# xiuqhou/Salience-DETR

Measured on AMD Instinct MI355X. Metric: images/s (whole node) + ms/encoder-layer, ResNet50 800x1333, higher is better.
Workload: dtype bf16; 1 GPU; salience_detr_resnet50_800_1333 bf16 inference, batch=2 per MI355X: pyramid flatten + hierarchical salience filtering + 6-layer salience encoder (MSDA); batch_per_gpu=2, global_batch=2, parallelism=replicas, images sharded across GPUs, no data-path collective, hipgraph=True, hipgraph_nodes=45, hipgraph_memset_nodes=0, world_size=1, backend=none (single process)

## Files before the change

include/salience_hip.h:

```cpp
#ifndef SALIENCE_HIP_H_
#define SALIENCE_HIP_H_

#include <stddef.h>
#include <stdint.h>

#ifdef __cplusplus
extern "C" {
#endif

typedef struct ihipStream_t *sdetr_stream_t;

#define SDETR_ABI_VERSION 1
#define SDETR_EINVAL (-1)

#define SDETR_F32 0
#define SDETR_BF16 1
#define SDETR_F16 2
#define SDETR_I64 3


int sdetr_abi_version(void);
const char *sdetr_last_error(void);

int sdetr_msda_im2col_f32(sdetr_stream_t stream, const float *data_value,
// ... 240 lines not shown
                                           int64_t mask_row_stride, const float *fill_value, int batch_size, int n, int k,
                                           int slices, int64_t index_offset, float *out_score, int64_t *out_index,
                                           int64_t out_row_stride, void *workspace, size_t workspace_bytes,
                                           const sdetr_rank_job *rank, const sdetr_finalize_job *finalize,
                                           int *jobs_carried);
int sdetr_stage1_x3_with_jobs(
    sdetr_stream_t stream, const float *x, int64_t x_batch_stride, int64_t x_row_stride, int batch_size, int tokens,
    int channels, const void *enc_weight_x3, const float *enc_bias, const float *enc_norm_weight,
    const float *enc_norm_bias, float enc_norm_eps, const float *row_scale, const float *coarse_score, int coarse_h,
    int coarse_w, int level_h, int level_w, const float *alpha, const float *norm_weight, const float *norm_bias,
    float norm_eps, const void *weight_x3, const float *bias, float *memory_out, int64_t memory_batch_stride,
    float *z_local, float *partial_sums, const void *vp_x, const void *vp_packed_weight, const float *vp_bias_padded,
    const uint8_t *vp_pad_mask, int vp_batch_size, int vp_spatial_size, int vp_num_heads, int vp_num_groups,
    void *vp_dst, int vp_dst_dtype, const sdetr_bordered_layout *vp_bordered, const sdetr_rank_job *rank,
    const sdetr_finalize_job *finalize);
int sdetr_salience_head_hoist_x3(
    sdetr_stream_t stream, const float *x, int64_t x_batch_stride, int64_t x_row_stride, int batch_size, int tokens,
    int channels, const void *enc_weight_x3, const float *enc_bias, const float *enc_norm_weight,
    const float *enc_norm_bias, float enc_norm_eps, const float *norm_weight, const void *weight_x3, float *memory_out,
    int64_t memory_batch_stride, float *g_out, int64_t g_batch_stride, float *sigma_out, int64_t sigma_batch_stride,
    const void *vp_x, const void *vp_packed_weight, const float *vp_bias_padded, const uint8_t *vp_pad_mask,
    int vp_batch_size, int vp_spatial_size, int vp_num_heads, int vp_num_groups, void *vp_dst, int vp_dst_dtype,
    const sdetr_bordered_layout *vp_bordered, const sdetr_finalize_job *finalize);
int sdetr_salience_head_modulate(sdetr_stream_t stream, const float *g, int64_t g_batch_stride, const float *sigma,
                                 int64_t sigma_batch_stride, int batch_size, int tokens, const float *row_scale,
                                 const float *coarse_score, int coarse_h, int coarse_w, int level_h, int level_w,
                                 const float *alpha, float norm_eps, const float *c0, float *z_local, float *partial_sums,
                                 const sdetr_rank_job *rank, const sdetr_finalize_job *finalize, float *score_min_init);
int sdetr_stage1_x3_with_value_proj(
    sdetr_stream_t stream, const float *x, int64_t x_batch_stride, int64_t x_row_stride, int batch_size, int tokens,
    int channels, const void *enc_weight_x3, const float *enc_bias, const float *enc_norm_weight,
    const float *enc_norm_bias, float enc_norm_eps, const float *row_scale, const float *coarse_score, int coarse_h,
    int coarse_w, int level_h, int level_w, const float *alpha, const float *norm_weight, const float *norm_bias,
    float norm_eps, const void *weight_x3, const float *bias, float *memory_out, int64_t memory_batch_stride,
    float *z_local, float *partial_sums, const void *vp_x, const void *vp_packed_weight, const float *vp_bias_padded,
    const uint8_t *vp_pad_mask, int vp_batch_size, int vp_spatial_size, int vp_num_heads, int vp_num_groups,
    void *vp_dst, int vp_dst_dtype, const sdetr_bordered_layout *vp_bordered);
int sdetr_salience_head_const(sdetr_stream_t stream, const float *partial_sums, int batch_size, int tokens,
                              const float *weight2, const float *bias2, float *const_workspace, float *score_min);
int sdetr_stage2_with_value_proj(sdetr_stream_t stream, const float *z_local, int batch_size, int tokens,
                                 const float *weight2_local_packed, const float *weight3_packed, const float *bias3,
                                 const float *weight4, const float *bias4, const float *const_workspace, float *score,
                                 float *score_flat, int64_t score_flat_stride, float *score_min, const void *vp_x,
                                 const void *vp_packed_weight, const float *vp_bias_padded, const uint8_t *vp_pad_mask,
                                 int vp_batch_size, int vp_spatial_size, int vp_num_heads, int vp_num_groups,
                                 void *vp_dst, int vp_dst_dtype, const sdetr_bordered_layout *vp_bordered,
// ... 340 lines not shown
```

salience_detr_amd/_hip.py:

```python
import ctypes
import os
import threading
from typing import Optional

import torch

_HERE = os.path.dirname(os.path.abspath(__file__))
LIB_PATH = os.path.join(_HERE, "libsalience_hip.so")
F16_LIB_PATH = os.path.join(_HERE, "libsalience_hip_f16.so")

F32, BF16, F16, I64 = 0, 1, 2, 3
EINVAL = -1
ACT16 = (torch.bfloat16, torch.float16)

_lib = None
_lib_f16 = None
_tls = threading.local()


def is_act16(dt) -> bool:
    return dt in ACT16

_i = ctypes.c_int

# ... 114 lines not shown
    "sdetr_pyramid_flatten": (_i, [_p, _i, _p, _p, _p, _p, _p, _p, _i, _i, _i, _p, _p, _p, _p, _p, _p, _p]),
    "sdetr_class_max_times": (_i, [_p, _p, _i, _p, _i64, _i, _i, _i, _p]),
    "sdetr_layernorm": (_i, [_p, _p, _p, _i, _i64, _i64, _i64, _i64, _p, _p, _p, _p, _i, ctypes.c_float, _i, _i, _i, _p, _i,
                             _p, _i64, _i]),
    "sdetr_advance_rows": (_i, [_p, _p, _p, _p, _p, _p, _i64, _p, _i, _i, _i, _i, _i, _i]),
    "sdetr_select_stack": (_i, [_p, _p, _i64, _p, _i64, _p, _i, _i, _i, _i, _p]),
    "sdetr_encoder_finalize_sorted": (_i, [_p, _p, _p, _p, _p, _p, _p, _i, _i, _i, _i, _i, _i, _p]),
    "sdetr_encoder_finalize": (_i, [_p, _p, _p, _p, _p, _p, _p, _i, _i, _i, _i, _i, _i, _p]),
    "sdetr_column_mean_f32": (_i, [_p, _p, _i64, _i64, _i, _i, _i, _p]),
    "sdetr_pack_linear_f32": (_i, [_p, _p, _i64, _i, _i, _p]),
    "sdetr_salience_head_blocks": (_i, [_i, _i]),
    "sdetr_salience_head_stage1": (_i, [_p, _p, _i64, _i64, _i, _i, _i, _p, _p, _p, _p, ctypes.c_float, _p, _p, _i, _i,
                                        _i, _i, _p, _p, _p, ctypes.c_float, _p, _p, _p, _i64, _p, _p]),
    "sdetr_salience_head_stage1_x3": (_i, [_p, _p, _i64, _i64, _i, _i, _i, _p, _p, _p, _p, ctypes.c_float, _p, _p, _i, _i,
                                        _i, _i, _p, _p, _p, ctypes.c_float, _p, _p, _p, _i64, _p, _p]),
    "sdetr_salience_head_const": (_i, [_p, _p, _i, _i, _p, _p, _p, _p]),
    "sdetr_stage2_with_value_proj": (_i, [_p, _p, _i, _i, _p, _p, _p, _p, _p, _p, _p, _p, _i64, _p,
                                          _p, _p, _p, _p, _i, _i, _i, _i, _p, _i, _p, _p, _p, _p, _p]),
    "sdetr_stage1_x3_with_value_proj": (_i, [_p, _p, _i64, _i64, _i, _i, _i, _p, _p, _p, _p, ctypes.c_float, _p, _p, _i, _i,
                                        _i, _i, _p, _p, _p, ctypes.c_float, _p, _p, _p, _i64, _p, _p,
                                             _p, _p, _p, _p, _i, _i, _i, _i, _p, _i, _p]),
    "sdetr_salience_head_hoist_x3": (_i, [_p, _p, _i64, _i64, _i, _i, _i, _p, _p, _p, _p, ctypes.c_float, _p, _p, _p, _i64, _p,
                                          _i64, _p, _i64, _p, _p, _p, _p, _i, _i, _i, _i, _p, _i, _p, _p]),
    "sdetr_salience_head_modulate": (_i, [_p, _p, _i64, _p, _i64, _i, _i, _p, _p, _i, _i, _i, _i, _p, ctypes.c_float, _p, _p, _p,
                                          _p, _p, _p]),
    "sdetr_stage1_x3_with_jobs": (_i, [_p, _p, _i64, _i64, _i, _i, _i, _p, _p, _p, _p, ctypes.c_float, _p, _p, _i, _i,
                                        _i, _i, _p, _p, _p, ctypes.c_float, _p, _p, _p, _i64, _p, _p,
                                             _p, _p, _p, _p, _i, _i, _i, _i, _p, _i, _p, _p, _p]),
    "sdetr_pack_linear_bf16x3": (_i, [_p, _p, _i64, _i, _i, _p]),
    "sdetr_salience_head_stage2": (_i, [_p, _p, _p, _i, _i, _p, _p, _p, _p, _p, _p, _p, _p, _p, _p, _i64, _p, _p, _i]),
    "sdetr_ffn_packed_bytes": (_i64, [_i]),
    "sdetr_ffn_pack_bf16": (_i, [_p, _p, _p, _i, _i, _p]),
    "sdetr_ffn_auto_splits": (_i, [_i, _i]),
    "sdetr_ffn_workspace_bytes": (_i64, [_i, _i]),
    "sdetr_ffn_fused_advance_bf16": (_i, [_p, _p, _p, _p, _p, _p, _p, ctypes.c_float, _i, _i, _i, _i, _i, _p, _i64, _p, _p, _p, _p,
                                          _i64, _p, _i, _i, _i]),
    "sdetr_attn_tail_packed_bytes": (_i64, []),
    "sdetr_attn_tail_pack_bf16": (_i, [_p, _p, _i, _p]),
    "sdetr_attn_tail_ffn_advance_bf16": (_i, [_p, _p, _p, _p, _p, _p, _p, ctypes.c_float, _p, _p, _p, _p, ctypes.c_float, _i, _i,
                                              _i, _i, _i, _p, _i64, _p, _p, _p, _p, _i64, _p, _i, _i, _i, _p, _p, _i64, _p]),
    "sdetr_class_head_packed_bytes": (_i64, []),
    "sdetr_class_head_pack_bf16": (_i, [_p, _p, _i, _i, _p]),
    "sdetr_gemm_x3_presplit": (_i, [_p, _p, _i64, _i, _i, _i, _p]),
    "sdetr_gemm_x3_f32": (_i, [_p, _p, _i64, _i, _p, _i64, _i, _p, _i64, _i, _i, _i, _p, _i, _p]),
    "sdetr_gemm_x3_epilogue_f32": (_i, [_p, _p, _i64, _i, _p, _i64, _i, _p, _i64, _i, _i, _i, _p, _i, _p, _i, _p, _i64]),
    "sdetr_topk_attention_with_projection_bf16": (_i, [_p, _p, _i64, _p, _i64, _p, _i, _i, _i, _p, _p, _p, _p, _p, _p,
# ... 125 lines not shown
```

salience_detr_amd/csrc/salience_head.hip:

```cpp
#include <cstdlib>

#include "common.h"

#include "salience_head_core.h"

namespace sdetr {

__global__ void __launch_bounds__(512, 2) salience_head_stage1_x3_kernel(Stage1Args p)
{
    stage1_x3_body(p, (int)blockIdx.x, (int)blockIdx.y);
}


template <int RT, int WAVES = 4>
__global__ void __launch_bounds__(64 * WAVES, WAVES == 8 ? 2 : (RT == 2 ? 2 : 4)) salience_head_stage1_kernel(Stage1Args p)
{
    constexpr int TM = 32 * RT, THREADS = 64 * WAVES, CT = 8 / WAVES;
    static_assert(TM * 64 % THREADS == 0 && THREADS % TM == 0, "tile / block shape");
    extern __shared__ __attribute__((aligned(16))) float smem[];
    float *tile = smem;
    float *par = smem + TM * kXS;
    float *srow = par + kParRows * kC;
    const int tid = threadIdx.x, lane = tid & 63, wave = tid >> 6;
    const int b = blockIdx.y, blk = blockIdx.x;
    const int t0 = blk * TM;
    const int nvalid = min(TM, p.n - t0);
    const int n0 = wave * (32 * CT);
    const bool with_enc = p.w_enc != nullptr;

    WeightStream<CT, 4> ws;
    ws.start(with_enc ? p.w_enc : p.w1, kC, kC / 8, n0, lane);

    {
        const float *xb = p.x + (int64_t)b * p.x_batch_stride + (int64_t)t0 * p.x_row_stride;
        constexpr int NL = TM * 64 / THREADS;
// ... 331 lines not shown
        return fail("salience_head_stage1_x3: NULL pointer");
    if (enc_weight_x3 && (!enc_bias || !enc_norm_weight || !enc_norm_bias))
        return fail("salience_head_stage1_x3: enc_output parameters incomplete");
    if (row_scale && coarse_score) return fail("salience_head_stage1_x3: give row_scale OR coarse_score");
    if (coarse_score && ((int64_t)level_h * level_w != tokens || coarse_h <= 0 || coarse_w <= 0))
        return fail("salience_head_stage1_x3: level %dx%d does not cover %d tokens", level_h, level_w, tokens);
    if ((x_row_stride % 4) || (x_batch_stride % 4)) return fail("salience_head_stage1_x3: rows must be 16-byte aligned");
    if (stage1_block_tokens(batch_size, tokens) != 32)
        return fail("salience_head_stage1_x3: 32-token blocks only (unset SDETR_HEAD_ROWTILES)");
    Stage1Args a;
    a.x = x; a.x_batch_stride = x_batch_stride; a.x_row_stride = x_row_stride;
    a.w_enc = reinterpret_cast<const float4 *>(enc_weight_x3);
    a.b_enc = enc_bias; a.g_enc = enc_norm_weight; a.beta_enc = enc_norm_bias; a.eps_enc = enc_norm_eps;
    a.row_scale = row_scale; a.coarse = coarse_score; a.ch = coarse_h; a.cw = coarse_w; a.h = level_h; a.w = level_w;
    a.alpha = alpha; a.g1 = norm_weight; a.beta1 = norm_bias; a.eps1 = norm_eps;
    a.w1 = reinterpret_cast<const float4 *>(weight_x3); a.b1 = bias;
    a.memory_out = enc_weight_x3 ? memory_out : nullptr; a.mem_batch_stride = memory_batch_stride;
    a.z_local = z_local; a.partial = partial_sums; a.n = tokens; a.nblk = (tokens + 31) / 32;
    hipLaunchKernelGGL(salience_head_stage1_x3_kernel, dim3((unsigned)a.nblk, (unsigned)batch_size), dim3(512),
                       (size_t)stage1_x3_lds_bytes(), static_cast<hipStream_t>(stream), a);
    return check_launch("salience_head_stage1_x3");
}

extern "C" int sdetr_salience_head_const(sdetr_stream_t stream, const float *partial_sums, int batch_size, int tokens,
                                         const float *weight2, const float *bias2, float *const_workspace,
                                         float *score_min)
{
    if (batch_size < 0 || tokens < 0) return fail("salience_head_const: negative size");
    if (batch_size == 0 || tokens == 0) return 0;
    if (!partial_sums || !weight2 || !bias2 || !const_workspace) return fail("salience_head_const: NULL pointer");
    hipLaunchKernelGGL(salience_head_const_kernel, dim3((unsigned)batch_size), dim3(kHalf * kConstGroups), 0,
                       static_cast<hipStream_t>(stream), partial_sums, sdetr_salience_head_blocks(batch_size, tokens),
                       tokens, weight2, bias2, const_workspace, score_min);
    return check_launch("salience_head_const");
}

extern "C" int sdetr_salience_head_stage2(sdetr_stream_t stream, const float *z_local, const float *partial_sums,
                                          int batch_size, int tokens, const float *weight2, const float *bias2,
                                          const float *weight2_local_packed, const float *weight3_packed,
                                          const float *bias3, const float *weight4, const float *bias4,
                                          float *const_workspace, float *score, float *score_flat,
                                          int64_t score_flat_stride, float *score_min, const void *weight2_local_x3,
                                          int const_in_block)
{
    if (batch_size < 0 || tokens < 0) return fail("salience_head_stage2: negative size");
    if (batch_size == 0 || tokens == 0) return 0;
// ... 27 lines not shown
```

salience_detr_amd/csrc/salience_head_core.h:

```cpp
#pragma once
#include "common.h"

#pragma clang fp contract(off)

namespace sdetr {

constexpr int kC = 256;
constexpr int kHalf = 128;
constexpr int kTM = 64;
constexpr int kXS = kC + 4;
constexpr int kZS = kHalf + 4;

using f32x16 = __attribute__((ext_vector_type(16))) float;

__device__ __forceinline__ float erf_pos(float t)
{
    float p = 4.535823973128572e-05f;
    p = fmaf(p, t, -0.00044550452730618417f);
    p = fmaf(p, t, 0.0014894308988004923f);
    p = fmaf(p, t, 0.0007746480405330658f);
    p = fmaf(p, t, -0.028253698721528053f);
    p = fmaf(p, t, 0.14848162233829498f);
    p = fmaf(p, t, 0.9184163808822632f);
    p = fmaf(p, t, 1.6279085874557495f);
// ... 295 lines not shown
                                                                     (int)((S + PD) * ws.kStep), 0);
        }
#pragma unroll
        for (int rt = 0; rt < RT; ++rt)
#pragma unroll
            for (int pl = 0; pl < 3; ++pl)
                a[rt][pl] = *reinterpret_cast<const u32x4_t *>(ap + rt * 32 * kRow + pl * kPlane + S * 32);
        __builtin_amdgcn_sched_barrier(0);
#pragma unroll
        for (int rt = 0; rt < RT; ++rt) {
            acc[rt] = mfma_bf16(a[rt][2], b[0], acc[rt]);
            acc[rt] = mfma_bf16(a[rt][0], b[2], acc[rt]);
            acc[rt] = mfma_bf16(a[rt][1], b[1], acc[rt]);
            acc[rt] = mfma_bf16(a[rt][1], b[0], acc[rt]);
            acc[rt] = mfma_bf16(a[rt][0], b[1], acc[rt]);
            acc[rt] = mfma_bf16(a[rt][0], b[0], acc[rt]);
        }
    }
}
constexpr int kS2PlaneRow = kHalf * 2 + 16;
constexpr int kS2PlaneBytes = 64 * kS2PlaneRow;
constexpr int kS2Planes = 3 * kS2PlaneBytes;

__device__ __forceinline__ void stage1_x3_body(const Stage1Args &p, int blk, int b)
{
    constexpr int TM = 32, THREADS = 512;
    extern __shared__ __attribute__((aligned(16))) float smem[];
    char *planes = reinterpret_cast<char *>(smem);
    float *tile = smem;
    float *par = smem + kX3Region / 4;
    float *srow = par + kParRows * kC;
    const int tid = threadIdx.x, lane = tid & 63;
    const int wave = __builtin_amdgcn_readfirstlane(tid >> 6);
    const int t0 = blk * TM;
    const int nvalid = min(TM, p.n - t0);
    const int n0 = wave * 32;
    const bool with_enc = p.w_enc != nullptr;
    const bool hoist = p.g_out != nullptr;

#ifdef SH_STAMPS
    long long sh_t[8];
    int sh_n = 0;
#define SH_STAMP() sh_t[sh_n++] = clock64()
#else
#define SH_STAMP()
#endif
    SH_STAMP();
    WeightStreamX3<kX3Depth> ws;
    ws.start(with_enc ? (const void *)p.w_enc : (const void *)p.w1, wave, lane);

    {
        const float *xb = p.x + (int64_t)b * p.x_batch_stride + (int64_t)t0 * p.x_row_stride;
        constexpr int NL = TM * 64 / THREADS;
        float4 v[NL];
#pragma unroll
        for (int i = 0; i < NL; ++i) {
            const int idx = tid + i * THREADS;
            const int r = idx >> 6, c4 = idx & 63;
            v[i] = *reinterpret_cast<const float4 *>(xb + (int64_t)min(r, nvalid - 1) * p.x_row_stride + c4 * 4);
        }
        if (tid < 256) {
            const int row = tid >> 6, c4 = tid & 63;
            const float *src0 = row == 0 ? p.b_enc : row == 1 ? p.g_enc : row == 2 ? p.beta_enc : p.g1;
            const float *src1 = row == 0 ? p.beta1 : p.b1;
            if (with_enc || row == 3) *reinterpret_cast<float4 *>(par + row * kC + c4 * 4) =
                                          *reinterpret_cast<const float4 *>(src0 + c4 * 4);
            if (row < 2) *reinterpret_cast<float4 *>(par + (4 + row) * kC + c4 * 4) =
                             *reinterpret_cast<const float4 *>(src1 + c4 * 4);
        }
        if (tid < TM) {
            float s = 0.f;
            const int t = min(t0 + tid, p.n - 1);
            if (p.row_scale) {
                s = p.row_scale[(int64_t)b * p.n + t];
            } else if (p.coarse) {
                const int y = t / p.w, x = t - y * p.w;
                const float sh = p.h > 1 ? (float)(p.ch - 1) / (float)(p.h - 1) : 0.f;
                const float sw = p.w > 1 ? (float)(p.cw - 1) / (float)(p.w - 1) : 0.f;
                const float fy = sh * (float)y, fx = sw * (float)x;
                const int y1 = (int)fy, x1 = (int)fx;
                const int yp = y1 < p.ch - 1 ? 1 : 0, xp = x1 < p.cw - 1 ? 1 : 0;
                const float ly = fy - (float)y1, lx = fx - (float)x1;
                const float hy = 1.f - ly, hx = 1.f - lx;
                const float *cm = p.coarse + (int64_t)b * p.ch * p.cw;
                s = hy * (hx * cm[y1 * p.cw + x1] + lx * cm[y1 * p.cw + x1 + xp]) +
                    ly * (hx * cm[(y1 + yp) * p.cw + x1] + lx * cm[(y1 + yp) * p.cw + x1 + xp]);
            }
            srow[tid] = s;
            if (tid == 0) srow[TM] = (p.row_scale || p.coarse) ? (p.alpha ? *p.alpha : 1.f) : 0.f;
        }
#pragma unroll
        for (int i = 0; i < NL; ++i) {
            const int idx = tid + i * THREADS;
            const int r = idx >> 6, c4 = idx & 63;
            const float4 val = r < nvalid ? v[i] : make_float4(0.f, 0.f, 0.f, 0.f);
#ifndef SH_SITE1_SOFT
#define SH_SITE1_SOFT false
#endif
#ifndef SH_SITE2_SOFT
#define SH_SITE2_SOFT false
#endif
            if (with_enc) store_split<SH_SITE1_SOFT>(planes, r, c4 * 4, val);
            else *reinterpret_cast<float4 *>(tile + r * kXS + c4 * 4) = val;
        }
    }
#ifdef SH_STAMPS
    asm volatile("s_waitcnt vmcnt(0) lgkmcnt(0)" ::: "memory");
    const long long sh_tile_done = clock64();
#endif
    __syncthreads();
    SH_STAMP();

    f32x16 acc;
    if (with_enc) {
#pragma unroll
        for (int i = 0; i < 16; ++i) acc[i] = 0.f;
        block_gemm_x3<kX3Depth>(planes, ws, lane, acc);
        SH_STAMP();
        ws.start(p.w1, wave, lane);
        __syncthreads();
        const int c = n0 + (lane & 31);
        const float bias = par[kParBEnc * kC + c];
#pragma unroll
        for (int i = 0; i < 16; ++i) tile[acc_row(i, lane) * kXS + c] = acc[i] + bias;
        __syncthreads();
        SH_STAMP();
    }

    {
        constexpr int TPR = THREADS / TM, NV = kC / 4 / TPR, CS = 4 * TPR;
        const int r = tid / TPR, q = tid % TPR;
        const float *row = tile + r * kXS + 4 * q;
// ... 14 lines not shown
            }
        }
        const float s = srow[r], a = srow[TM];
        if (a != 0.f) {
#pragma unroll
            for (int i = 0; i < NV; ++i)
                v[i] = make_float4(v[i].x + v[i].x * s * a, v[i].y + v[i].y * s * a, v[i].z + v[i].z * s * a,
                                   v[i].w + v[i].w * s * a);
        }
        row_stats<NV, TPR>(v, hoist ? 0.f : p.eps1, mean, rstd);
        if (hoist) {
            const bool flat = !(rstd < 3.0e38f);
            if (q == 0 && r < nvalid) p.sigma_out[(int64_t)b * p.sigma_batch_stride + t0 + r] = flat ? 0.f : 1.f / rstd;
            if (flat) rstd = 0.f;
        }
#ifndef SH_NO_PIN_STATS
        asm volatile("" : "+v"(mean), "+v"(rstd));
#endif
#pragma unroll
        for (int i = 0; i < NV; ++i)
            v[i] = ln_apply(v[i], mean, rstd, *reinterpret_cast<const float4 *>(par + kParG1 * kC + CS * i + 4 * q),
                            hoist ? make_float4(0.f, 0.f, 0.f, 0.f)
                                  : *reinterpret_cast<const float4 *>(par + kParBeta1 * kC + CS * i + 4 * q));
        __syncthreads();
#pragma unroll
        for (int i = 0; i < NV; ++i) store_split<SH_SITE2_SOFT>(planes, r, CS * i + 4 * q, v[i]);
    }
    __syncthreads();
    SH_STAMP();

#pragma unroll
    for (int i = 0; i < 16; ++i) acc[i] = 0.f;
    block_gemm_x3<kX3Depth>(planes, ws, lane, acc);
    SH_STAMP();
    if (hoist) {
        const int c = n0 + (lane & 31);
        float *g = p.g_out + (int64_t)b * p.g_batch_stride + (int64_t)t0 * kC + c;
#pragma unroll
        for (int i = 0; i < 16; ++i) {
            const int r = acc_row(i, lane);
            if (r < nvalid) g[(int64_t)r * kC] = acc[i];
        }
    } else {
        const int c = n0 + (lane & 31);
        const float bias = par[kParB1 * kC + c];
        if (n0 < kHalf) {
// ... 299 lines not shown
```

salience_detr_amd/filter_ops.py:

```python
import ctypes
import math
from typing import Optional

import torch
from torch import Tensor

from . import _hip
from .derived import derived


def masked_topk_desc(score: Tensor, k: int, mask: Optional[Tensor] = None, fill_with_global_min: bool = False,
                     payload: Optional[Tensor] = None, index_offset: int = 0, want_scores: bool = True,
                     fill_value: Optional[Tensor] = None, out=None, orders_job: Optional["RowOrdersJob"] = None,
                     carry_rank: Optional["RankJob"] = None, carry_finalize: Optional["FinalizeJob"] = None):
    _hip.require_device("masked_topk_desc", score=score, payload=payload, fill_value=fill_value)
    if score.dtype != torch.float32 or score.dim() != 2:
        raise RuntimeError("masked_topk_desc: score must be a 2-d float32 tensor")
    B, N = score.shape
    k = int(k)
    if k < 0 or k > N:
        raise RuntimeError(f"masked_topk_desc: selected index k out of range (k={k}, row length {N})")
    if mask is not None and not fill_with_global_min:
        raise RuntimeError("masked_topk_desc: a mask requires fill_with_global_min=True")
    if mask is None and payload is None and out is None and N > _SELECT_MAX_ROW and 0 < k <= 2048 and k * 16 <= N:
# ... 482 lines not shown
            if memory_out.shape != x.shape or memory_out.stride(2) != 1 or memory_out.stride(1) != C:
                raise RuntimeError("salience_head_hoist: memory_out must be [B,S,C] with contiguous rows")
            mbs = memory_out.stride(0)
    g = torch.empty((B, S, C), dtype=torch.float32, device=x.device)
    sigma = torch.empty((B, S), dtype=torch.float32, device=x.device)
    c0 = _layer1_constant(predictor)
    carry_value = value_job is not None and not value_job.done and value_job.value.device == x.device
    carry_fin = (finalize_job is not None and not finalize_job.done and not carry_value
                 and finalize_job.tokens.device == x.device)
    vp = value_job.pointers() if carry_value else (None, None, None, None, 0, 0, 0, 0, None, 0, None)
    fj = ctypes.byref(finalize_job.struct()) if carry_fin else None
    with torch.cuda.device(x.device):
        code = lib.sdetr_salience_head_hoist_x3(
            _hip.stream_ptr(), x.data_ptr(), x.stride(0), x.stride(1), B, S, C, _hip.ptr(w_enc), _hip.ptr(b_enc),
            _hip.ptr(g_enc), _hip.ptr(be_enc), eps_enc, l1n.weight.data_ptr(),
            packed_linear_weight(l1.weight, split3=True).data_ptr(), _hip.ptr(memory_out), mbs, g.data_ptr(), g.stride(0),
            sigma.data_ptr(), sigma.stride(0), *vp, fj)
    _hip.check(code, "salience_head_hoist")
    if carry_value:
        value_job.done = True
    if carry_fin:
        finalize_job.done = True
    return HoistedHead(g, sigma, c0)


def salience_head(x: Tensor, predictor, row_scale: Optional[Tensor] = None, coarse_score: Optional[Tensor] = None,
                  level_hw=None, alpha: Optional[Tensor] = None, enc_output=None, enc_output_norm=None,
                  memory_out: Optional[Tensor] = None, score_flat: Optional[Tensor] = None,
                  score_min: Optional[Tensor] = None, value_job: Optional[ValueProjectionJob] = None,
                  value_job2: Optional[ValueProjectionJob] = None, rank_job: Optional["RankJob"] = None,
                  finalize_job: Optional["FinalizeJob"] = None, hoisted: Optional["HoistedHead"] = None) -> Tensor:
    if not x.is_cuda:
        raise RuntimeError("salience_head: HIP device tensors required; there is no CPU fallback")
    if x.dtype != torch.float32 or x.dim() != 3 or x.stride(2) != 1:
        raise RuntimeError("salience_head: fp32 [B,n,C] with a contiguous last dim expected")
    B, n, C = x.shape
    job_act = next((j.value.dtype for j in (value_job, value_job2) if j is not None), None)
    if job_act is None and finalize_job is not None:
        job_act = finalize_job.tokens.dtype
    lib = _hip.lib(job_act)
    l1n, l1 = predictor.layer1[0], predictor.layer1[1]
    l2a, l2b, l2c = predictor.layer2[0], predictor.layer2[2], predictor.layer2[4]
    half = predictor.h_dim // 2
    if row_scale is not None:
        row_scale = row_scale.reshape(B, n)
        if row_scale.dtype != torch.float32 or not row_scale.is_contiguous():
# ... 1178 lines not shown
```

salience_detr_amd/hot_path.py:

```python
from typing import Optional, Sequence, Tuple

import torch
from torch import Tensor, nn

from . import _hip, pyramid
from .derived import derived
from .salience_encoder import SalienceTransformerEncoder, SalienceTransformerEncoderLayer
from .salience_filtering import MaskPredictor, level_filtering, salience_filtering, token_budgets


def filter_ops_bf16x3() -> bool:
    from . import filter_ops
    return bool(filter_ops.salience_head_bf16x3)


def resolve_activation_dtype(dtype: torch.dtype, value_dtype: Optional[torch.dtype] = None):
    if dtype == torch.float16:
        return dtype, (value_dtype or torch.float16)
    return dtype, value_dtype


class SalienceEncoderHotPath(nn.Module):
    def __init__(self, encoder: SalienceTransformerEncoder, num_classes: int, num_feature_levels: int = 4,
                 level_filter_ratio: Tuple = (0.25, 0.5, 1.0, 1.0),
# ... 32 lines not shown
        return self

    @property
    def encoder_dtype(self) -> torch.dtype:
        return self.encoder.layers[0].linear1.weight.dtype

    def _ratios(self):
        return derived(self, "ratios", (self.level_filter_ratio, self.layer_filter_ratio),
                       lambda: (tuple(self.level_filter_ratio.detach().cpu().tolist()),
                                tuple(self.layer_filter_ratio.detach().cpu().tolist())))

    value_projection_parts = (2, 1, 2, 1)
    value_projection_parts_hoisted = (3, 3)

    def forward(self, multi_level_feats: Sequence[Tensor], multi_level_masks: Sequence[Tensor],
                multi_level_pos_embeds: Sequence[Tensor],
                image_sizes: Optional[Sequence[Tuple[int, int]]] = None,
                canvas: Optional[Tuple[int, int]] = None, return_aux: bool = False):
        level_ratio, layer_ratio = self._ratios()
        edt = self.encoder_dtype
        native = not (torch.is_grad_enabled() and (any(p.requires_grad for p in self.parameters())
                                                   or any(f.requires_grad for f in multi_level_feats)))
        feat_enc = pos_enc = None
        if native and multi_level_feats[0].dtype == torch.float32:
            from .filter_ops import pyramid_flatten
            feat_flatten, lvl_pos_embed_flatten, enc_in, mask_flatten, feat_enc, pos_enc, valid_ratios_k = pyramid_flatten(
                multi_level_feats, multi_level_pos_embeds, multi_level_masks, self.level_embeds,
                want_bf16=(edt if _hip.is_act16(edt) else False), want_fp32=(return_aux or not _hip.is_act16(edt)))
        else:
            enc_in = valid_ratios_k = None
            feat_flatten = pyramid.flatten_multi_level(multi_level_feats)
            mask_flatten = pyramid.flatten_multi_level(multi_level_masks)
            lvl_pos_embed_flatten = pyramid.get_lvl_pos_embed(self.level_embeds.to(multi_level_pos_embeds[0].dtype),
                                                              multi_level_pos_embeds)
        value_maps = None
        value_jobs = None
        if native and feat_enc is not None and self.fuse_value_projection:
            n_layers = len(self.encoder.layers)
            from . import salience_filtering as _sf
            hoisted = _sf.HOIST_HEAD and filter_ops_bf16x3()
            parts = ((self.value_projection_parts_hoisted if hoisted else self.value_projection_parts) if n_layers == 6
                     else min(3 if hoisted else 4, n_layers))
            plan = self.encoder.plan_values(feat_enc, mask_flatten, parts=parts,
                                            level_shapes=pyramid.level_shapes_of(multi_level_masks))
            if plan is not None:
                value_maps, value_jobs = plan
        level_shapes = pyramid.level_shapes_of(multi_level_masks)
        finalize_job = None
        if native and feat_enc is not None and self.fuse_value_projection:
            finalize_job = self.encoder.plan_finalize(feat_enc, mask_flatten, level_shapes)
        if valid_ratios_k is not None:
            spatial_shapes, level_start_index = pyramid.shape_tensors(level_shapes, mask_flatten.device)
            valid_ratios = valid_ratios_k
        else:
            spatial_shapes, level_start_index, valid_ratios = pyramid.multi_level_misc(multi_level_masks)
        starts = [0]
        for h, w in level_shapes[:-1]:
            starts.append(starts[-1] + h * w)

        fuse_enc = (enc_in is not None and self.enc_mask_predictor.fused_kernels_apply(enc_in)
                    and self.enc_output.weight.dtype == torch.float32)
        backbone_output_memory = None
        if fuse_enc:
            if return_aux:
                backbone_output_memory = torch.empty_like(enc_in)
        elif enc_in is not None:
            from .filter_ops import fused_layer_norm
            backbone_output_memory = fused_layer_norm(self.enc_output(enc_in), self.enc_output_norm)
        else:
            backbone_output_memory = pyramid.encoder_output_memory(
                self.enc_output, self.enc_output_norm, feat_flatten + lvl_pos_embed_flatten, mask_flatten,
                level_shapes)

        if image_sizes is not None:
            if canvas is None:
                raise ValueError("image_sizes needs the padded canvas size as well")
            def build():
                focus_host, level_host, _ = pyramid.host_token_budgets(image_sizes, canvas, level_shapes, level_ratio)
                return (torch.as_tensor(focus_host, dtype=torch.int64).to(mask_flatten.device),
                        [int(v) for v in level_host])
            focus_token_nums, level_token_nums = pyramid.static_tensor(
                ("budgets", tuple(map(tuple, image_sizes)), tuple(canvas), tuple(level_shapes), level_ratio,
                 str(mask_flatten.device)), build)
        else:
            focus_token_nums, level_dev, _ = token_budgets(multi_level_masks, self.level_filter_ratio.float())
            level_token_nums = level_dev.tolist()
            focus_token_nums = focus_token_nums.to(torch.int64)

        score_flat = None
        extras: dict = {}
        if fuse_enc:
            score_flat = torch.empty(mask_flatten.shape, dtype=torch.float32, device=mask_flatten.device)
            salience_score, level_inds, level_score = level_filtering(
                enc_in, mask_flatten, level_shapes, starts, level_token_nums, self.enc_mask_predictor, self.alpha,
                enc_output=self.enc_output, enc_output_norm=self.enc_output_norm, memory_out=backbone_output_memory,
                score_flat=score_flat, extras=extras, value_jobs=value_jobs, finalize_job=finalize_job)
        else:
            salience_score, level_inds, level_score = level_filtering(
                backbone_output_memory, mask_flatten, level_shapes, starts, level_token_nums, self.enc_mask_predictor,
                self.alpha)
        foreground_inds, foreground_score = salience_filtering(salience_score, level_inds, level_score, mask_flatten,
                                                               layer_ratio, score_flat=score_flat, extras=extras,
                                                               lazy_foreground=native and not return_aux)
        if feat_enc is None:
            feat_enc, pos_enc = feat_flatten.to(edt), lvl_pos_embed_flatten.to(edt)
        for job in value_jobs or ():
            job.run()
        memory = self.encoder(
            precomputed_value_maps=value_maps, query=feat_enc, query_pos=pos_enc, query_key_padding_mask=mask_flatten,
            spatial_shapes=spatial_shapes, level_start_index=level_start_index, valid_ratios=valid_ratios,
            foreground_score=foreground_score, focus_token_nums=focus_token_nums, foreground_inds=foreground_inds,
            multi_level_masks=multi_level_masks, finalize_job=finalize_job)
        if not return_aux:
            return memory, salience_score
        aux = dict(feat_flatten=feat_flatten, mask_flatten=mask_flatten, lvl_pos_embed_flatten=lvl_pos_embed_flatten,
                   spatial_shapes=spatial_shapes, level_start_index=level_start_index, valid_ratios=valid_ratios,
                   backbone_output_memory=backbone_output_memory, focus_token_nums=focus_token_nums,
                   level_token_nums=level_token_nums, level_inds=level_inds, level_score=level_score,
                   foreground_inds=foreground_inds, foreground_score=foreground_score)
# ... 13 lines not shown
```

salience_detr_amd/salience_filtering.py:

```python
from typing import List, Optional, Sequence, Tuple

import torch
from torch import Tensor, nn
from torch.nn import functional as F

from . import pyramid
from .layer_norm_train import add_layer_norm
from .salience_encoder import split_prefix
from . import filter_ops
from .filter_ops import (column_mean, fused_layer_norm, masked_fill_min, masked_topk_desc, merge_sorted_desc,
                         plan_masked_topk, salience_head, salience_head_hoist)

HOIST_HEAD = True
HOIST_CARRIES_VALUE = False
FINALIZE_LEVEL = "merge"
RANK_ON_MERGE = True


class _Modulate(torch.autograd.Function):

    @staticmethod
    def forward(ctx, x, row_scale, alpha):
        ctx.save_for_backward(x, row_scale, alpha)
        return torch.addcmul(x, x, row_scale.unsqueeze(-1) * alpha)
# ... 98 lines not shown
        h = F.gelu(h)
        h = F.gelu(self.layer2[2](h))
        return self.layer2[4](h)


def token_budgets(multi_level_masks: Sequence[Tensor], level_filter_ratio: Tensor):
    valid = torch.stack([(~m).sum((1, 2)) for m in multi_level_masks], -1)
    focus = (valid * level_filter_ratio).int()
    return focus.sum(-1), focus.max(0)[0], valid


def _next_value_jobs(value_jobs, stage2_only=None) -> dict:
    if stage2_only is not None:
        pending = [j for j in stage2_only if not j.done]
        return dict(value_job=None, value_job2=pending[0] if pending else None)
    pending = [j for j in (value_jobs or ()) if not j.done]
    return dict(value_job=pending[0] if pending else None, value_job2=pending[1] if len(pending) > 1 else None)


def level_filtering(backbone_output_memory: Tensor, mask_flatten: Tensor, level_shapes: Sequence[Tuple[int, int]],
                    level_start_index: Sequence[int], level_token_nums: Sequence[int], mask_predictor: nn.Module,
                    alpha: Tensor, enc_output: Optional[nn.Module] = None, enc_output_norm: Optional[nn.Module] = None,
                    memory_out: Optional[Tensor] = None, score_flat: Optional[Tensor] = None,
                    extras: Optional[dict] = None, value_jobs: Optional[list] = None, finalize_job=None):
    B = backbone_output_memory.shape[0]
    L = len(level_shapes)
    salience_score: List[Optional[Tensor]] = [None] * L
    level_inds: List[Optional[Tensor]] = [None] * L
    level_score: List[Optional[Tensor]] = [None] * L
    score = None
    fused = (isinstance(mask_predictor, MaskPredictor) and backbone_output_memory.is_cuda
             and mask_predictor.fused_kernels_apply(backbone_output_memory)
             and not (torch.is_grad_enabled() and (backbone_output_memory.requires_grad or alpha.requires_grad or
                                                   any(p.requires_grad for p in mask_predictor.parameters()))))
    if enc_output is not None and not fused:
        raise RuntimeError("level_filtering: enc_output fusion needs the no-grad fp32 256-wide MaskPredictor path")
    level_min = sel_score = sel_inds = None
    pending_rank = None
    defer_ranks = fused
    if fused:
        dev = backbone_output_memory.device
        level_min = torch.empty(L, dtype=torch.float32, device=dev)
        ks = [int(k) for k in level_token_nums]
        offs = [sum(ks[:i]) for i in range(L)]
        sel_score = torch.empty((B, sum(ks)), dtype=torch.float32, device=dev)
        sel_inds = torch.empty((B, sum(ks)), dtype=torch.int64, device=dev)
    hoisted = None
    if fused and HOIST_HEAD and filter_ops.salience_head_bf16x3:
        pending = [j for j in (value_jobs or ()) if not j.done]
        hoisted = salience_head_hoist(backbone_output_memory, mask_predictor, enc_output=enc_output,
                                      enc_output_norm=enc_output_norm, memory_out=memory_out,
                                      value_job=pending[0] if pending and HOIST_CARRIES_VALUE else None,
                                      finalize_job=finalize_job if FINALIZE_LEVEL is None else None)
    fin_level = FINALIZE_LEVEL if isinstance(FINALIZE_LEVEL, int) else (-1 if FINALIZE_LEVEL == "merge" else 0)
    for lvl in range(L - 1, -1, -1):
        h, w = level_shapes[lvl]
        start = int(level_start_index[lvl])
        level_memory = backbone_output_memory[:, start:start + h * w, :]
        mask = mask_flatten[:, start:start + h * w]
        if fused and hoisted is not None:
            token_score = salience_head(
                level_memory, mask_predictor, coarse_score=score, level_hw=(h, w),
                alpha=alpha[lvl:lvl + 1] if score is not None else None,
                score_flat=None if score_flat is None else score_flat[:, start:start + h * w],
                score_min=level_min[lvl:lvl + 1],
                rank_job=pending_rank if lvl > 0 or not RANK_ON_MERGE else None,
                finalize_job=finalize_job if lvl <= fin_level else None,
                hoisted=hoisted.level(start, h * w),
                **_next_value_jobs(None, stage2_only=value_jobs if lvl >= L - 3 and L > 3 and value_jobs else None))
        elif fused:
            token_score = salience_head(
# ... 76 lines not shown
```

Measured before the change: 2007 images/s.

## Fuse pyramid flatten into the hoisted salience head stage-1 kernel

```diff
diff --git a/include/salience_hip.h b/include/salience_hip.h
--- a/include/salience_hip.h
+++ b/include/salience_hip.h
@@ -286,6 +286,13 @@
     const void *vp_x, const void *vp_packed_weight, const float *vp_bias_padded, const uint8_t *vp_pad_mask,
     int vp_batch_size, int vp_spatial_size, int vp_num_heads, int vp_num_groups, void *vp_dst, int vp_dst_dtype,
     const sdetr_bordered_layout *vp_bordered, const sdetr_finalize_job *finalize);
+int sdetr_salience_head_hoist_pyramid_x3(
+    sdetr_stream_t stream, int num_levels, const float *const *feats, const float *const *pos, const uint8_t *const *masks,
+    const int *heights, const int *widths, const float *level_embeds, int batch_size, int channels, int spatial_size,
+    uint8_t *mask_out, void *feat_act, void *pos_act, float *valid_ratios, const void *enc_weight_x3, const float *enc_bias,
+    const float *enc_norm_weight, const float *enc_norm_bias, float enc_norm_eps, const float *norm_weight,
+    const void *weight_x3, float *memory_out, int64_t memory_batch_stride, float *g_out, int64_t g_batch_stride,
+    float *sigma_out, int64_t sigma_batch_stride);
 int sdetr_salience_head_modulate(sdetr_stream_t stream, const float *g, int64_t g_batch_stride, const float *sigma,
                                  int64_t sigma_batch_stride, int batch_size, int tokens, const float *row_scale,
                                  const float *coarse_score, int coarse_h, int coarse_w, int level_h, int level_w,
diff --git a/salience_detr_amd/_hip.py b/salience_detr_amd/_hip.py
--- a/salience_detr_amd/_hip.py
+++ b/salience_detr_amd/_hip.py
@@ -160,6 +160,8 @@
                                              _p, _p, _p, _p, _i, _i, _i, _i, _p, _i, _p]),
     "sdetr_salience_head_hoist_x3": (_i, [_p, _p, _i64, _i64, _i, _i, _i, _p, _p, _p, _p, ctypes.c_float, _p, _p, _p, _i64, _p,
                                           _i64, _p, _i64, _p, _p, _p, _p, _i, _i, _i, _i, _p, _i, _p, _p]),
+    "sdetr_salience_head_hoist_pyramid_x3": (_i, [_p, _i, _p, _p, _p, _p, _p, _p, _i, _i, _i, _p, _p, _p, _p, _p, _p, _p, _p,
+                                                  ctypes.c_float, _p, _p, _p, _i64, _p, _i64, _p, _i64]),
     "sdetr_salience_head_modulate": (_i, [_p, _p, _i64, _p, _i64, _i, _i, _p, _p, _i, _i, _i, _i, _p, ctypes.c_float, _p, _p, _p,
                                           _p, _p, _p]),
     "sdetr_stage1_x3_with_jobs": (_i, [_p, _p, _i64, _i64, _i, _i, _i, _p, _p, _p, _p, ctypes.c_float, _p, _p, _i, _i,
diff --git a/salience_detr_amd/csrc/salience_head.hip b/salience_detr_amd/csrc/salience_head.hip
--- a/salience_detr_amd/csrc/salience_head.hip
+++ b/salience_detr_amd/csrc/salience_head.hip
@@ -11,6 +11,11 @@
     stage1_x3_body(p, (int)blockIdx.x, (int)blockIdx.y);
 }
 
+__global__ void __launch_bounds__(512, 2) salience_head_hoist_pyramid_kernel(Stage1Args p, PyramidSrc src, int s1_blocks)
+{
+    const int blk = (int)blockIdx.x;
+    stage1_x3_body<true>(p, blk % s1_blocks, blk / s1_blocks, &src);
+}
 
 template <int RT, int WAVES = 4>
 __global__ void __launch_bounds__(64 * WAVES, WAVES == 8 ? 2 : (RT == 2 ? 2 : 4)) salience_head_stage1_kernel(Stage1Args p)
@@ -388,6 +393,68 @@
     return check_launch("salience_head_stage1_x3");
 }
 
+extern "C" int sdetr_salience_head_hoist_pyramid_x3(
+    sdetr_stream_t stream, int num_levels, const float *const *feats, const float *const *pos, const uint8_t *const *masks,
+    const int *heights, const int *widths, const float *level_embeds, int batch_size, int channels, int spatial_size,
+    uint8_t *mask_out, void *feat_act, void *pos_act, float *valid_ratios, const void *enc_weight_x3, const float *enc_bias,
+    const float *enc_norm_weight, const float *enc_norm_bias, float enc_norm_eps, const float *norm_weight,
+    const void *weight_x3, float *memory_out, int64_t memory_batch_stride, float *g_out, int64_t g_batch_stride,
+    float *sigma_out, int64_t sigma_batch_stride)
+{
+    if (num_levels <= 0 || num_levels > kPyrMaxLevels) return fail("salience_head_hoist_pyramid_x3: 1..%d levels", kPyrMaxLevels);
+    if (channels != kC) return fail("salience_head_hoist_pyramid_x3: built for embed_dim = hidden_dim = %d (got %d)", kC, channels);
+    if (batch_size < 0 || spatial_size <= 0) return fail("salience_head_hoist_pyramid_x3: bad dims");
+    if (!feats || !pos || !masks || !heights || !widths || !level_embeds || !mask_out || !feat_act || !pos_act)
+        return fail("salience_head_hoist_pyramid_x3: null pointer");
+    if (!enc_weight_x3 || !enc_bias || !enc_norm_weight || !enc_norm_bias || !norm_weight || !weight_x3 || !g_out || !sigma_out)
+        return fail("salience_head_hoist_pyramid_x3: null pointer (head)");
+    if ((g_batch_stride % 4) || g_batch_stride < (int64_t)spatial_size * kC || sigma_batch_stride < spatial_size ||
+        (memory_out && ((memory_batch_stride % 4) || memory_batch_stride < (int64_t)spatial_size * kC)))
+        return fail("salience_head_hoist_pyramid_x3: bad output batch strides");
+    if (stage1_block_tokens(batch_size, spatial_size) != 32)
+        return fail("salience_head_hoist_pyramid_x3: 32-token blocks only (unset SDETR_HEAD_ROWTILES)");
+    PyramidSrc src{};
+    src.levels = num_levels;
+    int64_t start = 0;
+    for (int l = 0; l < num_levels; ++l) {
+        const int H = heights[l], W = widths[l];
+        if (H <= 0 || W <= 0 || !feats[l] || !pos[l] || !masks[l]) return fail("salience_head_hoist_pyramid_x3: bad level %d", l);
+        src.feat[l] = feats[l]; src.pos[l] = pos[l]; src.mask[l] = masks[l];
+        src.H[l] = H; src.W[l] = W; src.start[l] = (int)start;
+        src.box_wh[l] = 0.05f * (float)(1u << l);
+        start += (int64_t)H * W;
+        if (start > spatial_size || (int64_t)batch_size * kC * H * W > 0x7fffffffffffLL)
+            return fail("salience_head_hoist_pyramid_x3: sizes out of range");
+    }
+    if (start != spatial_size)
+        return fail("salience_head_hoist_pyramid_x3: spatial_size %d is not the pixel count %lld", spatial_size, (long long)start);
+    for (int l = num_levels; l <= kPyrMaxLevels; ++l) src.start[l] = spatial_size;
+    for (int l = 0; l + kPyrTileLevels < num_levels; ++l)
+        if (src.start[l + kPyrTileLevels] / 32 == (src.start[l + 1] - 1) / 32)
+            return fail("salience_head_hoist_pyramid_x3: more than %d levels inside one 32-token tile", kPyrTileLevels);
+    if (batch_size == 0) return 0;
+    src.level_embed = level_embeds;
+    src.feat_act = reinterpret_cast<bf16_t *>(feat_act); src.pos_act = reinterpret_cast<bf16_t *>(pos_act);
+    src.mask_out = mask_out; src.valid_ratios = valid_ratios;
+    Stage1Args a;
+    a.x = nullptr; a.x_batch_stride = 0; a.x_row_stride = 0;
+    a.w_enc = reinterpret_cast<const float4 *>(enc_weight_x3);
+    a.b_enc = enc_bias; a.g_enc = enc_norm_weight; a.beta_enc = enc_norm_bias; a.eps_enc = enc_norm_eps;
+    a.row_scale = nullptr; a.coarse = nullptr; a.ch = a.cw = a.h = a.w = 0;
+    a.alpha = nullptr; a.g1 = norm_weight; a.beta1 = norm_weight; a.eps1 = 0.f;
+    a.w1 = reinterpret_cast<const float4 *>(weight_x3); a.b1 = norm_weight;
+    a.memory_out = memory_out; a.mem_batch_stride = memory_batch_stride;
+    a.z_local = nullptr; a.partial = nullptr; a.n = spatial_size; a.nblk = (spatial_size + 31) / 32;
+    a.g_out = g_out; a.g_batch_stride = g_batch_stride; a.sigma_out = sigma_out; a.sigma_batch_stride = sigma_batch_stride;
+    if ((int64_t)a.nblk * batch_size > 0x7fffffff) return fail("salience_head_hoist_pyramid_x3: too many tiles");
+    static DeviceOnce lds_once;
+    const int lds = kPyrLdsFloats * (int)sizeof(float);
+    allow_dynamic_lds(salience_head_hoist_pyramid_kernel, lds_once, lds);
+    hipLaunchKernelGGL(salience_head_hoist_pyramid_kernel, dim3((unsigned)(a.nblk * batch_size)), dim3(512), (size_t)lds,
+                       static_cast<hipStream_t>(stream), a, src, a.nblk);
+    return check_launch("salience_head_hoist_pyramid_x3");
+}
+
 extern "C" int sdetr_salience_head_const(sdetr_stream_t stream, const float *partial_sums, int batch_size, int tokens,
                                          const float *weight2, const float *bias2, float *const_workspace,
                                          float *score_min)
diff --git a/salience_detr_amd/csrc/salience_head_core.h b/salience_detr_amd/csrc/salience_head_core.h
--- a/salience_detr_amd/csrc/salience_head_core.h
+++ b/salience_detr_amd/csrc/salience_head_core.h
@@ -341,14 +341,35 @@
 constexpr int kS2PlaneBytes = 64 * kS2PlaneRow;
 constexpr int kS2Planes = 3 * kS2PlaneBytes;
 
-__device__ __forceinline__ void stage1_x3_body(const Stage1Args &p, int blk, int b)
+constexpr int kPyrMaxLevels = 8;
+constexpr int kPyrTileLevels = 4;
+struct PyramidSrc {
+    const float *feat[kPyrMaxLevels], *pos[kPyrMaxLevels];
+    const uint8_t *mask[kPyrMaxLevels];
+    int H[kPyrMaxLevels], W[kPyrMaxLevels], start[kPyrMaxLevels + 1];
+    float box_wh[kPyrMaxLevels];
+    const float *level_embed;
+    int levels;
+    bf16_t *feat_act, *pos_act;
+    uint8_t *mask_out;
+    float *valid_ratios;
+};
+constexpr int kPyrGeo = 8;
+constexpr int kPyrLdsFloats = 2 * 32 * kXS + kParRows * kC + 32 + 4 + kPyrTileLevels * kC + kPyrTileLevels * kPyrGeo + 32 * 4;
+
+template <bool PYR = false>
+__device__ __forceinline__ void stage1_x3_body(const Stage1Args &p, int blk, int b, const PyramidSrc *src = nullptr)
 {
     constexpr int TM = 32, THREADS = 512;
     extern __shared__ __attribute__((aligned(16))) float smem[];
     char *planes = reinterpret_cast<char *>(smem);
     float *tile = smem;
-    float *par = smem + kX3Region / 4;
+    float *par = smem + (PYR ? 2 * TM * kXS : kX3Region / 4);
     float *srow = par + kParRows * kC;
+    float *tpos = smem + TM * kXS;
+    float *lemb = srow + TM + 4;
+    float *geo = lemb + kPyrTileLevels * kC;
+    int *rowinfo = reinterpret_cast<int *>(geo + kPyrTileLevels * kPyrGeo);
     const int tid = threadIdx.x, lane = tid & 63;
     const int wave = __builtin_amdgcn_readfirstlane(tid >> 6);
     const int t0 = blk * TM;
@@ -368,15 +389,69 @@
     WeightStreamX3<kX3Depth> ws;
     ws.start(with_enc ? (const void *)p.w_enc : (const void *)p.w1, wave, lane);
 
+    int l0 = 0;
     {
-        const float *xb = p.x + (int64_t)b * p.x_batch_stride + (int64_t)t0 * p.x_row_stride;
         constexpr int NL = TM * 64 / THREADS;
         float4 v[NL];
+        constexpr int NC = kC * TM / THREADS;
+        float pf[NC], pq[NC];
+        const int tok = tid & 31, cg = tid >> 5;
+        if (PYR) {
+            const PyramidSrc &s = *src;
+            for (int j = 1; j < s.levels; ++j) l0 += t0 >= s.start[j] ? 1 : 0;
+            const int t = min(t0 + tok, p.n - 1);
+            int slot = 0, wl = s.W[l0], hw = s.H[l0] * s.W[l0], st = s.start[l0];
+            const float *fp = s.feat[l0], *pp = s.pos[l0];
+            const uint8_t *mp = s.mask[l0];
+#pragma unroll
+            for (int k = 1; k < kPyrTileLevels; ++k) {
+                const int l = min(l0 + k, s.levels - 1);
+                if (l0 + k < s.levels && t >= s.start[l]) {
+                    slot = k; wl = s.W[l]; hw = s.H[l] * s.W[l]; st = s.start[l];
+                    fp = s.feat[l]; pp = s.pos[l]; mp = s.mask[l];
+                }
+            }
+            const int tl = t - st;
+            const int64_t e0 = ((int64_t)b * kC + cg) * hw + tl;
+#pragma unroll
+            for (int i = 0; i < NC; ++i) pf[i] = fp[e0 + (int64_t)(i * (THREADS / TM)) * hw];
+#pragma unroll
+            for (int i = 0; i < NC; ++i) pq[i] = pp[e0 + (int64_t)(i * (THREADS / TM)) * hw];
+            if (tid < TM) {
+                const int y = tl / wl;
+                *reinterpret_cast<int4 *>(rowinfo + 4 * tok) = make_int4(slot, tl - y * wl, y, (int)mp[(int64_t)b * hw + tl]);
+            }
+            {
+                const int l = l0 + (wave >> 1);
+                if (l < s.levels && s.start[l] < t0 + TM) {
+                    const int H = s.H[l], W = s.W[l];
+                    const uint8_t *mb = s.mask[l] + (int64_t)b * H * W;
+                    int cnt = 0;
+                    if (wave & 1) { for (int i = lane; i < W; i += 64) cnt += mb[i] == 0; }
+                    else          { for (int i = lane; i < H; i += 64) cnt += mb[(int64_t)i * W] == 0; }
+#pragma unroll
+                    for (int o = 32; o > 0; o >>= 1) cnt += __shfl_xor(cnt, o);
+                    if (lane == 0) {
+                        float *g = geo + (wave >> 1) * kPyrGeo;
+                        g[wave & 1] = (float)cnt;
+                        if (!(wave & 1)) { g[2] = (float)H; g[3] = (float)W; g[4] = s.box_wh[l]; }
+                    }
+                }
+            }
+            if (tid >= 256) {
+                const int l = l0 + ((tid - 256) >> 6), c4 = tid & 63;
+                if (l < s.levels)
+                    *reinterpret_cast<float4 *>(lemb + ((tid - 256) >> 6) * kC + c4 * 4) =
+                        *reinterpret_cast<const float4 *>(s.level_embed + (int64_t)l * kC + c4 * 4);
+            }
+        } else {
+        const float *xb = p.x + (int64_t)b * p.x_batch_stride + (int64_t)t0 * p.x_row_stride;
 #pragma unroll
         for (int i = 0; i < NL; ++i) {
             const int idx = tid + i * THREADS;
             const int r = idx >> 6, c4 = idx & 63;
             v[i] = *reinterpret_cast<const float4 *>(xb + (int64_t)min(r, nvalid - 1) * p.x_row_stride + c4 * 4);
+        }
         }
         if (tid < 256) {
             const int row = tid >> 6, c4 = tid & 63;
@@ -408,8 +483,15 @@
             srow[tid] = s;
             if (tid == 0) srow[TM] = (p.row_scale || p.coarse) ? (p.alpha ? *p.alpha : 1.f) : 0.f;
         }
-#pragma unroll
-        for (int i = 0; i < NL; ++i) {
+        if (PYR) {
+#pragma unroll
+            for (int i = 0; i < NC; ++i) {
+                tile[tok * kXS + cg + i * (THREADS / TM)] = pf[i];
+                tpos[tok * kXS + cg + i * (THREADS / TM)] = pq[i];
+            }
+        }
+#pragma unroll
+        for (int i = 0; i < (PYR ? 0 : NL); ++i) {
             const int idx = tid + i * THREADS;
             const int r = idx >> 6, c4 = idx & 63;
             const float4 val = r < nvalid ? v[i] : make_float4(0.f, 0.f, 0.f, 0.f);
@@ -427,6 +509,45 @@
     asm volatile("s_waitcnt vmcnt(0) lgkmcnt(0)" ::: "memory");
     const long long sh_tile_done = clock64();
 #endif
+    if (PYR) {
+        __syncthreads();
+        const PyramidSrc &s = *src;
+        const int r = tid >> 4, q = tid & 15;
+        const int4 ri = *reinterpret_cast<const int4 *>(rowinfo + 4 * r);
+        const float *g = geo + ri.x * kPyrGeo;
+        const float vh = g[0], vw = g[1], box_wh = g[4];
+        const bool pad = ri.w != 0;
+        const float cx = ((float)ri.y + 0.5f) / vw, cy = ((float)ri.z + 0.5f) / vh;
+        const bool keep = !pad && cx > 0.01f && cx < 0.99f && cy > 0.01f && cy < 0.99f && box_wh > 0.01f && box_wh < 0.99f;
+        const bool live = r < nvalid;
+        const int64_t o = ((int64_t)b * p.n + t0 + r) * kC + 4 * q;
+        float4 sum[4];
+#pragma unroll
+        for (int i = 0; i < 4; ++i) {
+            const int c = 64 * i + 4 * q;
+            const float4 fv = *reinterpret_cast<const float4 *>(tile + r * kXS + c);
+            const float4 pv = *reinterpret_cast<const float4 *>(tpos + r * kXS + c);
+            const float4 e = *reinterpret_cast<const float4 *>(lemb + ri.x * kC + c);
+            const float4 qv = make_float4(pv.x + e.x, pv.y + e.y, pv.z + e.z, pv.w + e.w);
+            sum[i] = keep && live ? make_float4(fv.x + qv.x, fv.y + qv.y, fv.z + qv.z, fv.w + qv.w)
+                                  : make_float4(0.f, 0.f, 0.f, 0.f);
+            if (live) {
+                *reinterpret_cast<uint2 *>(s.feat_act + o + 64 * i) = make_uint2(pack_act2(fv.x, fv.y), pack_act2(fv.z, fv.w));
+                *reinterpret_cast<uint2 *>(s.pos_act + o + 64 * i) = make_uint2(pack_act2(qv.x, qv.y), pack_act2(qv.z, qv.w));
+            }
+        }
+        if (live && q == 0) {
+            s.mask_out[(int64_t)b * p.n + t0 + r] = pad ? 1 : 0;
+            if (s.valid_ratios && ri.y == 0 && ri.z == 0) {
+                float *vr = s.valid_ratios + ((int64_t)b * s.levels + l0 + ri.x) * 2;
+                vr[0] = vw / g[3];
+                vr[1] = vh / g[2];
+            }
+        }
+        __syncthreads();
+#pragma unroll
+        for (int i = 0; i < 4; ++i) store_split<SH_SITE1_SOFT>(planes, r, 64 * i + 4 * q, sum[i]);
+    }
     __syncthreads();
     SH_STAMP();
 
@@ -487,6 +608,8 @@
             v[i] = ln_apply(v[i], mean, rstd, *reinterpret_cast<const float4 *>(par + kParG1 * kC + CS * i + 4 * q),
                             hoist ? make_float4(0.f, 0.f, 0.f, 0.f)
                                   : *reinterpret_cast<const float4 *>(par + kParBeta1 * kC + CS * i + 4 * q));
+        asm volatile("s_waitcnt lgkmcnt(0)" ::: "memory");
+        __builtin_amdgcn_sched_barrier(0);
         __syncthreads();
 #pragma unroll
         for (int i = 0; i < NV; ++i) store_split<SH_SITE2_SOFT>(planes, r, CS * i + 4 * q, v[i]);
diff --git a/salience_detr_amd/filter_ops.py b/salience_detr_amd/filter_ops.py
--- a/salience_detr_amd/filter_ops.py
+++ b/salience_detr_amd/filter_ops.py
@@ -528,6 +528,76 @@
     if carry_fin:
         finalize_job.done = True
     return HoistedHead(g, sigma, c0)
+
+
+FLATTEN_IN_STAGE1 = True
+_PYR_TILE_LEVELS = 4
+
+
+def hoist_pyramid_applies(multi_level_feats, multi_level_pos_embeds, multi_level_masks, predictor, enc_output, act) -> bool:
+    feats, L = list(multi_level_feats), len(multi_level_feats)
+    if not (FLATTEN_IN_STAGE1 and salience_head_bf16x3 and _hip.is_act16(act) and 1 <= L <= 8):
+        return False
+    if any((not t.is_cuda) or t.dtype != torch.float32 or t.dim() != 4 or t.shape[1] != 256
+           for t in feats + list(multi_level_pos_embeds)):
+        return False
+    if any(m.dtype not in (torch.bool, torch.uint8) for m in multi_level_masks):
+        return False
+    if not (getattr(predictor, "h_dim", 0) == 256 and predictor.layer1[1].weight.dtype == torch.float32
+            and enc_output is not None and enc_output.weight.dtype == torch.float32 and enc_output.weight.is_cuda):
+        return False
+    starts = [0]
+    for f in feats:
+        starts.append(starts[-1] + int(f.shape[2]) * int(f.shape[3]))
+    return all(starts[l + _PYR_TILE_LEVELS] // 32 != (starts[l + 1] - 1) // 32 for l in range(L - _PYR_TILE_LEVELS))
+
+
+def salience_head_hoist_pyramid(multi_level_feats, multi_level_pos_embeds, multi_level_masks, level_embeds: Tensor, predictor,
+                                enc_output, enc_output_norm, act: torch.dtype, memory_out: Optional[Tensor] = None):
+    feats = [f.contiguous() for f in multi_level_feats]
+    pos = [p.contiguous() for p in multi_level_pos_embeds]
+    masks = [m.contiguous() for m in multi_level_masks]
+    _hip.require_device("salience_head_hoist_pyramid", level_embeds=level_embeds, **{f"feat{i}": f for i, f in enumerate(feats)},
+                        **{f"pos{i}": t for i, t in enumerate(pos)}, **{f"mask{i}": m for i, m in enumerate(masks)})
+    if not hoist_pyramid_applies(feats, pos, masks, predictor, enc_output, act):
+        raise RuntimeError("salience_head_hoist_pyramid: fp32 [B,256,H,W] maps, a 16-bit activation type and the fp32 256-wide "
+                           "head on the bf16x3 kernels expected (at most 8 levels, at most 4 inside one 32-token tile)")
+    L = len(feats)
+    B, C = feats[0].shape[:2]
+    for f, q, m in zip(feats, pos, masks):
+        if q.shape != f.shape or tuple(m.shape) != (B, f.shape[2], f.shape[3]) or f.shape[:2] != (B, C):
+            raise RuntimeError("salience_head_hoist_pyramid: feature / position / mask shapes of a level disagree")
+    S = sum(int(f.shape[2]) * int(f.shape[3]) for f in feats)
+    dev = feats[0].device
+    mask_out = torch.empty((B, S), dtype=torch.bool, device=dev)
+    feat_act = torch.empty((B, S, C), dtype=act, device=dev)
+    pos_act = torch.empty((B, S, C), dtype=act, device=dev)
+    valid_ratios = torch.empty((B, L, 2), dtype=torch.float32, device=dev)
+    le = level_embeds.detach().float().contiguous()
+    g = torch.empty((B, S, C), dtype=torch.float32, device=dev)
+    sigma = torch.empty((B, S), dtype=torch.float32, device=dev)
+    mbs = 0
+    if memory_out is not None:
+        if memory_out.shape != g.shape or memory_out.stride(2) != 1 or memory_out.stride(1) != C or memory_out.dtype != torch.float32:
+            raise RuntimeError("salience_head_hoist_pyramid: memory_out must be fp32 [B,S,C] with contiguous rows")
+        mbs = memory_out.stride(0)
+    l1n, l1 = predictor.layer1[0], predictor.layer1[1]
+    c0 = _layer1_constant(predictor)
+    mu8s = [m.view(torch.uint8) if m.dtype == torch.bool else m for m in masks]
+    ptrs = lambda ts: (ctypes.c_void_p * L)(*[t.data_ptr() for t in ts])
+    ints = lambda vs: (ctypes.c_int * L)(*vs)
+    lib = _hip.lib(act)
+    with torch.cuda.device(dev):
+        code = lib.sdetr_salience_head_hoist_pyramid_x3(
+            _hip.stream_ptr(), L, ptrs(feats), ptrs(pos), ptrs(mu8s), ints([int(f.shape[2]) for f in feats]),
+            ints([int(f.shape[3]) for f in feats]), le.data_ptr(), B, C, S, mask_out.data_ptr(), feat_act.data_ptr(),
+            pos_act.data_ptr(), valid_ratios.data_ptr(), packed_linear_weight(enc_output.weight, split3=True).data_ptr(),
+            enc_output.bias.detach().data_ptr(), enc_output_norm.weight.detach().data_ptr(),
+            enc_output_norm.bias.detach().data_ptr(), float(enc_output_norm.eps), l1n.weight.data_ptr(),
+            packed_linear_weight(l1.weight, split3=True).data_ptr(), _hip.ptr(memory_out), mbs, g.data_ptr(), g.stride(0),
+            sigma.data_ptr(), sigma.stride(0))
+    _hip.check(code, "salience_head_hoist_pyramid")
+    return HoistedHead(g, sigma, c0), mask_out, feat_act, pos_act, valid_ratios
 
 
 def salience_head(x: Tensor, predictor, row_scale: Optional[Tensor] = None, coarse_score: Optional[Tensor] = None,
diff --git a/salience_detr_amd/hot_path.py b/salience_detr_amd/hot_path.py
--- a/salience_detr_amd/hot_path.py
+++ b/salience_detr_amd/hot_path.py
@@ -78,7 +78,17 @@
         native = not (torch.is_grad_enabled() and (any(p.requires_grad for p in self.parameters())
                                                    or any(f.requires_grad for f in multi_level_feats)))
         feat_enc = pos_enc = None
-        if native and multi_level_feats[0].dtype == torch.float32:
+        hoisted_head = None
+        from . import filter_ops, salience_filtering as _sf
+        if (native and not return_aux and multi_level_feats[0].dtype == torch.float32 and _sf.HOIST_HEAD
+                and not _sf.HOIST_CARRIES_VALUE and _sf.FINALIZE_LEVEL is not None
+                and filter_ops.hoist_pyramid_applies(multi_level_feats, multi_level_pos_embeds, multi_level_masks,
+                                                     self.enc_mask_predictor, self.enc_output, edt)):
+            enc_in = feat_flatten = lvl_pos_embed_flatten = None
+            hoisted_head, mask_flatten, feat_enc, pos_enc, valid_ratios_k = filter_ops.salience_head_hoist_pyramid(
+                multi_level_feats, multi_level_pos_embeds, multi_level_masks, self.level_embeds, self.enc_mask_predictor,
+                self.enc_output, self.enc_output_norm, edt)
+        elif native and multi_level_feats[0].dtype == torch.float32:
             from .filter_ops import pyramid_flatten
             feat_flatten, lvl_pos_embed_flatten, enc_in, mask_flatten, feat_enc, pos_enc, valid_ratios_k = pyramid_flatten(
                 multi_level_feats, multi_level_pos_embeds, multi_level_masks, self.level_embeds,
@@ -114,8 +124,8 @@
         for h, w in level_shapes[:-1]:
             starts.append(starts[-1] + h * w)
 
-        fuse_enc = (enc_in is not None and self.enc_mask_predictor.fused_kernels_apply(enc_in)
-                    and self.enc_output.weight.dtype == torch.float32)
+        fuse_enc = hoisted_head is not None or (enc_in is not None and self.enc_mask_predictor.fused_kernels_apply(enc_in)
+                                                and self.enc_output.weight.dtype == torch.float32)
         backbone_output_memory = None
         if fuse_enc:
             if return_aux:
@@ -148,9 +158,10 @@
         if fuse_enc:
             score_flat = torch.empty(mask_flatten.shape, dtype=torch.float32, device=mask_flatten.device)
             salience_score, level_inds, level_score = level_filtering(
-                enc_in, mask_flatten, level_shapes, starts, level_token_nums, self.enc_mask_predictor, self.alpha,
-                enc_output=self.enc_output, enc_output_norm=self.enc_output_norm, memory_out=backbone_output_memory,
-                score_flat=score_flat, extras=extras, value_jobs=value_jobs, finalize_job=finalize_job)
+                enc_in if hoisted_head is None else hoisted_head.g, mask_flatten, level_shapes, starts, level_token_nums,
+                self.enc_mask_predictor, self.alpha, enc_output=self.enc_output, enc_output_norm=self.enc_output_norm,
+                memory_out=backbone_output_memory, score_flat=score_flat, extras=extras, value_jobs=value_jobs,
+                finalize_job=finalize_job, hoisted=hoisted_head)
         else:
             salience_score, level_inds, level_score = level_filtering(
                 backbone_output_memory, mask_flatten, level_shapes, starts, level_token_nums, self.enc_mask_predictor,
diff --git a/salience_detr_amd/salience_filtering.py b/salience_detr_amd/salience_filtering.py
--- a/salience_detr_amd/salience_filtering.py
+++ b/salience_detr_amd/salience_filtering.py
@@ -144,7 +144,8 @@
                     level_start_index: Sequence[int], level_token_nums: Sequence[int], mask_predictor: nn.Module,
                     alpha: Tensor, enc_output: Optional[nn.Module] = None, enc_output_norm: Optional[nn.Module] = None,
                     memory_out: Optional[Tensor] = None, score_flat: Optional[Tensor] = None,
-                    extras: Optional[dict] = None, value_jobs: Optional[list] = None, finalize_job=None):
+                    extras: Optional[dict] = None, value_jobs: Optional[list] = None, finalize_job=None,
+                    hoisted=None):
     B = backbone_output_memory.shape[0]
     L = len(level_shapes)
     salience_score: List[Optional[Tensor]] = [None] * L
@@ -167,8 +168,9 @@
         offs = [sum(ks[:i]) for i in range(L)]
         sel_score = torch.empty((B, sum(ks)), dtype=torch.float32, device=dev)
         sel_inds = torch.empty((B, sum(ks)), dtype=torch.int64, device=dev)
-    hoisted = None
-    if fused and HOIST_HEAD and filter_ops.salience_head_bf16x3:
+    if hoisted is not None and not fused:
+        raise RuntimeError("level_filtering: a hoisted head needs the no-grad fp32 256-wide MaskPredictor path")
+    if hoisted is None and fused and HOIST_HEAD and filter_ops.salience_head_bf16x3:
         pending = [j for j in (value_jobs or ()) if not j.done]
         hoisted = salience_head_hoist(backbone_output_memory, mask_predictor, enc_output=enc_output,
                                       enc_output_norm=enc_output_norm, memory_out=memory_out,
```

Result: faster. 2069 images/s, median of 6 (+3.1%).
